# plouj/eraytracer

Measured on AMD Instinct MI355X. Metric: Mpixels/sec at 4096x4096, recursion depth 5 (frame rendered into HBM, gathered to rank 0), higher is better.
Workload: dtype f64; 1 GPU; S64 4096x4096 depth 5; scene=s64, spp=1, width=4096, height=4096, depth=5, order=exact, framebuffer=f32, row_block=16, inflight=4, engine=wave, parallelism=rows1, world_size=1, rccl_ranks=1, hw_queues=4, spheres=64, triangles=0

## Files before the change

### eraytracer_amd/csrc/rt_render.hip

```cpp
#pragma clang fp contract(off)

#include <hip/hip_runtime.h>

#include <chrono>
#include <cmath>
#include <cstddef>
#include <cstdio>
#include <cstdlib>
#include <cstring>
#include <algorithm>
#include <mutex>
#include <type_traits>
#include <vector>

#include "../../include/rt_mi355x.h"
#include "rt_layout.h"
#include "rt_internal.h"
#include "rt_scene.h"

using namespace rtl;

namespace {

constexpr int BLOCK = 256;
// ... 437 lines not shown

}

size_t rt_trim(rt_prepared *p) {
    if (!p) return 0;
    DevGuard g(p->device);
    const size_t freed = free_work(p);
    p->pmask_valid = false;
    ++p->gen;
    return freed;
}

namespace {

size_t queue_budget() {
    static size_t b = [] {
        const char *s = std::getenv("RT_QUEUE_MB");
        size_t mb = s ? std::strtoull(s, nullptr, 10) : 8192;
        return (mb < 64 ? 64 : mb) << 20;
    }();
    return b;
}

bool lit_overlap(const rt_prepared *p) {
    static bool env_on = [] {
        const char *s = std::getenv("RT_LIT_STREAM");
        return !(s && std::strcmp(s, "0") == 0);
    }();
    return p->side_mode < 0 ? env_on : p->side_mode != 0;
}

int side_stream(rt_prepared *p, int depth) {
    if (!p->side[0]) {
        int least = 0, greatest = 0;
        HIPCHK(hipDeviceGetStreamPriorityRange(&least, &greatest));
        for (hipStream_t &x : p->side) HIPCHK(hipStreamCreateWithPriority(&x, hipStreamNonBlocking, least));
    }
    while (p->ev_level.size() < (size_t)depth + 1) {
        hipEvent_t a = nullptr, b = nullptr;
        HIPCHK(hipEventCreateWithFlags(&a, hipEventDisableTiming));
        if (hipEventCreateWithFlags(&b, hipEventDisableTiming) != hipSuccess) {
            (void)hipEventDestroy(a);
            return RT_EHIP;
        }
        p->ev_level.push_back(a);
        p->ev_lit.push_back(b);
    }
    return RT_OK;
}

size_t valid_slab_rows(int H, int rb, int sh, int ns) {
    const size_t slab = rt_shard_rows((uint32_t)H, (uint32_t)rb, (uint32_t)ns);
    size_t v = 0;
    for (size_t blk = 0; blk * rb < slab; ++blk) {
        const long long base = ((long long)blk * ns + sh) * rb;
        v += (size_t)std::max(0LL, std::min((long long)rb, (long long)H - base));
    }
    return v;
}

bool wave_single_write(const rt_prepared *p, int D, bool levels) {
    const int nrefl = (p->hdr.n_light > 0 && D > 1) ? D - 1 : 0;
    const bool overlap = lit_overlap(p) && D > 1 && p->hdr.n_light > 0;
    return nrefl == 0 || (!overlap && !levels);
}

template <int PREC, bool GENPOW>
int launch_wavefront(rt_prepared *p, int W, int H, int D, int rb, int sh, int ns, int row_begin, int row_end, void *out,
                     uint8_t *levels, hipStream_t st, int spp = 1, int sample = 0, unsigned long long seed = 0,
                     double *acc = nullptr, int levels_hit = 0) {
    uint8_t *const levels_primary = levels;
    if (levels_hit) levels = nullptr;
    const int slab_rows = row_end - row_begin;
    const int nlev = D > 0 ? D : 1;
    const size_t per_row = (size_t)W * nlev * sizeof(HitRec);
    int pass_rows = (int)std::min<size_t>((size_t)slab_rows, std::max<size_t>(TILE, queue_budget() / per_row));
    pass_rows = std::max(TILE, pass_rows / TILE * TILE);
    if (pass_rows > slab_rows) pass_rows = slab_rows;
    const int tiles_x = (W + TILE - 1) / TILE;
    const size_t max_tiles = (size_t)tiles_x * ((pass_rows + TILE - 1) / TILE);
    const size_t slots = max_tiles * TILE_SLOTS;
    int rc = grow(p, rt_prepared::W_QUEUE, slots * nlev * sizeof(HitRec));
    const size_t col_doubles = slots * COL_W * (size_t)std::max(1, nlev - 1);
    if (rc == RT_OK) rc = grow(p, rt_prepared::W_COLBUF, col_doubles * sizeof(double));
    if (rc == RT_OK) rc = grow(p, rt_prepared::W_CHILD, slots * nlev);
    if (rc == RT_OK) rc = grow(p, rt_prepared::W_LIT, slots * nlev * sizeof(unsigned));
    if (rc == RT_OK) rc = grow(p, rt_prepared::W_COUNTS, max_tiles * nlev * sizeof(int));
    const bool overlap = lit_overlap(p) && D > 1 && p->hdr.n_light > 0;
    const size_t list0 = level_counts(nlev);
    const size_t items_ints = list0 + slots * nlev;
    if (rc == RT_OK) rc = grow(p, rt_prepared::W_ITEMS, items_ints * sizeof(int));
    if (rc == RT_OK && overlap) rc = side_stream(p, D);
    if (rc != RT_OK) return rc;
    const unsigned long long *pmask = nullptr;
    if (p->hdr.beam_ok && D > 0) {
        const int slab_all = (int)rt_shard_rows(H, rb, ns);
        const size_t nhalf = (size_t)tiles_x * ((slab_all + TILE - 1) / TILE) * 2;
        const long long key[8] = {W, H, rb, sh, ns, spp > 1, (long long)p->scene_gen, slab_all};
        if (!(p->pmask_valid && std::memcmp(key, p->pmask_key, sizeof(key)) == 0)) {
            p->pmask_valid = false;
            ++p->gen;
            if ((rc = grow(p, rt_prepared::W_PMASK, nhalf * p->hdr.n_chunk * 8)) != RT_OK) return rc;
            const dim3 pg((unsigned)std::min<size_t>(4096, (nhalf + 3) / 4));
            KtScope kt(p, RT_KT_PMASK, st);
            with_bool(spp > 1, [&](auto ss) {
                hipLaunchKernelGGL(k_pmask<decltype(ss)::value>, pg, dim3(256), 0, st, p->hdr, p->d_tab, p->d_itab, W, H,
                                   rb, sh, ns, slab_all, (int)nhalf, p->buf<unsigned long long>(rt_prepared::W_PMASK));
            });
            HIPCHK(hipGetLastError());
            std::memcpy(p->pmask_key, key, sizeof(key));
            p->pmask_valid = true;
        }
        pmask = p->buf<unsigned long long>(rt_prepared::W_PMASK);
    }
    auto ls = [&](int k) { return overlap ? p->side[std::min(k, 1)] : st; };
    HitRec *const q = p->buf<HitRec>(rt_prepared::W_QUEUE);
    double *const d_colbuf = p->buf<double>(rt_prepared::W_COLBUF);
    uint8_t *const d_child = p->buf<uint8_t>(rt_prepared::W_CHILD);
    unsigned *const d_lit = p->buf<unsigned>(rt_prepared::W_LIT);
    int *const d_counts = p->buf<int>(rt_prepared::W_COUNTS);
    int *const d_items = p->buf<int>(rt_prepared::W_ITEMS);
    const int nrefl = (p->hdr.n_light > 0 && D > 1) ? D - 1 : 0;
    const int nshade = D > 0 ? 1 + nrefl : 0;
    const bool sph_only = p->hdr.n_tri == 0 && p->hdr.n_pl == 0 && p->hdr.cull_ok && p->hdr.occ_ok;
    const bool staged = sph_only && p->hdr.l_bytes > 0;
    const size_t lds = staged ? (size_t)p->hdr.l_bytes : 0;
    SceneHdr rhdr = p->hdr;
    size_t lds_bvh = lds;
    if (rhdr.bvh_ok) {
        const size_t nb = (size_t)rhdr.n_bvh * BVH_NODE_DOUBLES * 8, sb = (size_t)rhdr.n_sph * SPH_W * 8;
        if (nb + sb <= (size_t)BVH_LDS_MAX) {
            rhdr.l_bvh = (int)lds_bvh;
            rhdr.l_bsph = (int)(lds_bvh + nb);
            lds_bvh += nb + sb;
        }
        rhdr.l_stack = (int)lds_bvh;
        lds_bvh += (size_t)BLOCK * rhdr.bvh_depth * sizeof(unsigned);
    }
    auto bvh_at = [&](int k) { return !staged && rhdr.bvh_ok && k >= rhdr.bvh_level; };
    auto lds_r = [&](int k) { return bvh_at(k) ? lds_bvh : lds; };
    const bool fuse = !overlap && !levels && nrefl > 0;
    const bool iw = fuse && p->hdr.n_light <= 32 && nrefl >= 2;
    for (int row0 = row_begin; row0 < row_end; row0 += pass_rows) {
        const int rows = std::min(pass_rows, row_end - row0);
        const int ntiles = tiles_x * ((rows + TILE - 1) / TILE);
        const size_t off = (size_t)row0 * W;
        void *o = static_cast<char *>(out) + off * 3 * (PREC == RT_OUT_F64 ? 8 : 4);
        uint8_t *lv = levels ? levels + off : nullptr;
        uint8_t *lv0 = levels_primary ? levels_primary + off : nullptr;
        double *acc_p = acc ? acc + off * 3 : nullptr;
        auto qk = [&](int k) { return q + (size_t)k * ntiles * TILE_SLOTS; };
        auto ck = [&](int k) { return d_counts + (size_t)k * ntiles; };
        int *nitems = d_items;
        int *lists = d_items + list0;
        auto ik = [&](int k) { return lists + (size_t)k * ntiles * TILE_SLOTS; };
        auto colk = [&](int k) { return k > 0 ? d_colbuf + (size_t)(k - 1) * ntiles * TILE_SLOTS * COL_W : nullptr; };
        auto chk = [&](int k) { return d_child + (size_t)k * ntiles * TILE_SLOTS; };
        auto litk = [&](int k) { return d_lit + (size_t)k * ntiles * TILE_SLOTS; };
        const dim3 iblocks((ntiles + ITEMS_BLOCK - 1) / ITEMS_BLOCK);
        const PassGeom g{W, H, rb, sh, ns, row0, spp, sample, seed, acc_p};
        const dim3 grid(std::min(ntiles, PRIMARY_GRID));
        {
            KtScope kt(p, RT_KT_PRIMARY, st);
            with_bool(lv0 != nullptr, [&](auto has_lv) {
                hipLaunchKernelGGL((k_primary<PREC, decltype(has_lv)::value>), grid, dim3(PRIMARY_BLOCK), 0, st, p->hdr,
                                   p->d_tab, p->d_itab, W, H, D, rb, sh, ns, rows, row0, o, lv0, q, d_counts, ntiles, spp,
                                   sample, seed, acc_p, pmask, nitems);
            });
        }
        HIPCHK(hipGetLastError());
        const int sblocks = std::min<int>(STRIDE_BLOCKS, (ntiles * (TILE_SLOTS / 64) + BLOCK / 64 - 1) / (BLOCK / 64));
        const int sblocks1 = std::min<int>(STRIDE_BLOCKS_L1, (ntiles * (TILE_SLOTS / 64) + BLOCK / 64 - 1) / (BLOCK / 64));
        const int sblocksw = std::min<int>(STRIDE_BLOCKS_WALK, (ntiles * (TILE_SLOTS / 64) + BLOCK / 64 - 1) / (BLOCK / 64));
        const int sblocksb = std::min<int>(STRIDE_BLOCKS_BVH, (ntiles * (TILE_SLOTS / 64) + BLOCK / 64 - 1) / (BLOCK / 64));
        auto level_lists = [&](int k) -> int {
            if (iw && k == nrefl) return RT_OK;
            hipLaunchKernelGGL(k_items, iblocks, dim3(ITEMS_BLOCK), 0, st, ck(k), ntiles, ik(k), nitems + k);
            HIPCHK(hipGetLastError());
            if (overlap) {
                HIPCHK(hipEventRecord(p->ev_level[k], st));
                HIPCHK(hipStreamWaitEvent(ls(k), p->ev_level[k], 0));
            }
            if (fuse && k < nrefl) return RT_OK;
            if (k == nrefl && k >= 2) {
                if (overlap) HIPCHK(hipEventRecord(p->ev_lit[k], ls(k)));
                return RT_OK;
            }
            const int lblocks = k >= 2 ? std::min(sblocks, DEEP_LIGHT_BLOCKS) : sblocks;
            with_sph(staged, sph_only, [&](auto sph) {
                hipLaunchKernelGGL((k_light<PREC, GENPOW, decltype(sph)::value>), dim3(lblocks), dim3(BLOCK), lds, ls(k),
                                   p->hdr, p->d_tab, p->d_itab, k, o, qk(k), ik(k), nitems + k, colk(k), litk(k), g);
            });
            HIPCHK(hipGetLastError());
            if (overlap) HIPCHK(hipEventRecord(p->ev_lit[k], ls(k)));
            return RT_OK;
        };
        if (nshade > 0 && (rc = level_lists(0)) != RT_OK) return rc;
        for (int k = 1; k <= nrefl; ++k) {
            KtScope kt(p, k == 1 ? RT_KT_LEVEL1 : 0, st);
            if (fuse) {
                const bool bvh_k = bvh_at(k), ilp = bvh_k || k != 1, last = ilp && iw && k == nrefl;
                with_sph(staged, sph_only, [&](auto sph) {
                    constexpr int SPH = decltype(sph)::value;
                    auto rs = [&](auto ilp_c, auto bvh_c, auto last_c) {
                        constexpr bool BVH = decltype(bvh_c)::value;
                        hipLaunchKernelGGL(
                            (k_reflect_shade<PREC, GENPOW, SPH, decltype(ilp_c)::value, BVH, decltype(last_c)::value>),
                            dim3(k == 1 ? sblocks1 : BVH ? sblocksb : sblocks), dim3(BLOCK), lds_r(k), st, rhdr, p->d_tab,
                            p->d_itab, k, o, qk(k - 1), ik(k - 1), nitems + (k - 1), qk(k), ck(k), iw ? nullptr : chk(k - 1),
                            colk(k - 1), g, iw && k >= 2 ? (k == nrefl ? 2 : 1) : 0);
                    };
                    auto rs_ilp = [&](auto bvh_c) {
                        with_bool(last, [&](auto last_c) { rs(std::true_type{}, bvh_c, last_c); });
                    };
                    if (!ilp) rs(std::false_type{}, std::false_type{}, std::false_type{});
                    else if constexpr (SPH == 2) rs_ilp(std::false_type{});
                    else with_bool(bvh_k, rs_ilp);
                });
            } else {
                with_bool(lv != nullptr, [&](auto has_lv) {
                    with_bool(k != 1, [&](auto ilp_c) {
                        hipLaunchKernelGGL((k_reflect<decltype(has_lv)::value, decltype(ilp_c)::value>), dim3(sblocks),
                                           dim3(BLOCK), lds, st, rhdr, p->d_tab, p->d_itab, k, qk(k - 1), ik(k - 1),
                                           nitems + (k - 1), qk(k), ck(k), lv, chk(k - 1), g);
                    });
                });
            }
            HIPCHK(hipGetLastError());
            if ((rc = level_lists(k)) != RT_OK) return rc;
        }
        if (nrefl > 0) {
            const size_t ls_ = (size_t)ntiles * TILE_SLOTS;
            const bool bits = p->hdr.n_light <= 32;
            auto walk = [&](hipStream_t s_, int lo, int hi, bool deep) {
                with_sph(staged, sph_only, [&](auto sph) {
                    with_bool(bits, [&](auto bits_c) {
                        auto launch = [&](auto deep_c, auto pad_c) {
                            hipLaunchKernelGGL((k_walk<PREC, GENPOW, decltype(sph)::value, decltype(bits_c)::value,
                                                       decltype(deep_c)::value, decltype(pad_c)::value>),
                                               dim3(sblocksw), dim3(BLOCK), lds, s_, p->hdr, p->d_tab, p->d_itab, D, o, q,
                                               ls_, lists, nitems, d_colbuf, d_child, d_lit, lo, hi, g);
                        };
                        if (deep && fuse && bits) launch(std::true_type{}, std::true_type{});
                        else if (deep) launch(std::true_type{}, std::false_type{});
                        else launch(std::false_type{}, std::false_type{});
                    });
                });
            };
            if (overlap) {
                HIPCHK(hipStreamWaitEvent(p->side[0], p->ev_lit[1], 0));
                if (D > 2) HIPCHK(hipStreamWaitEvent(p->side[0], p->ev_level[2], 0));
                walk(p->side[0], 1, 2, false);
                HIPCHK(hipGetLastError());
                HIPCHK(hipEventRecord(p->ev_lit[0], p->side[0]));
            }
            if (D > 2 && overlap) {
                with_sph(staged, sph_only, [&](auto sph) {
                    hipLaunchKernelGGL((k_walk_deep<GENPOW, decltype(sph)::value>), dim3(sblocks), dim3(BLOCK), lds, st,
                                       p->hdr, p->d_tab, p->d_itab, D, q, ls_, lists, nitems, d_child, colk(2));
                });
                HIPCHK(hipGetLastError());
            }
            if (overlap) {
                HIPCHK(hipStreamWaitEvent(st, p->ev_lit[nrefl], 0));
                HIPCHK(hipStreamWaitEvent(st, p->ev_lit[0], 0));
                if (D > 2) walk(st, 2, D, false);
            } else if (!iw) {
                walk(st, 1, D, true);
            }
            HIPCHK(hipGetLastError());
        } else if (overlap && nshade > 0) {
            HIPCHK(hipStreamWaitEvent(st, p->ev_lit[0], 0));
        }
    }
    return RT_OK;
}

bool graphs_on() {
    static bool on = [] {
        const char *s = std::getenv("RT_GRAPH");
        return s && std::strcmp(s, "1") == 0;
    }();
    return on;
}

template <typename F>
int launch_frame(rt_prepared *p, const long long (&args)[12], hipStream_t st, F &&enqueue) {
    hipStreamCaptureStatus cs = hipStreamCaptureStatusNone;
    if (!graphs_on() || hipStreamIsCapturing(st, &cs) != hipSuccess || cs != hipStreamCaptureStatusNone)
        return enqueue(st);
    long long key[12];
    std::memcpy(key, args, sizeof(key));
    key[11] = (long long)p->gen;
// ... 184 lines not shown
```

### eraytracer_amd/csrc/rt_shade.inc

```

#ifndef RT_MAX_GROUPS
#define RT_MAX_GROUPS 3
#endif
constexpr int MAX_GROUPS = RT_MAX_GROUPS;
constexpr int UNION_CHUNKS = 4;
template <bool PRE, bool ILP = false, int SPH = 0, bool NB = false>
__device__ __forceinline__ int nearest(const Scene &S, int org, const D3 &o, const D3 &d, double &bt, bool act,
                                       int grp = -1, bool bvh = false) {
    const SceneHdr &h = S.h;
    bt = __builtin_inf();
    int bid = 0x7fffffff;
    if (__ballot(act) == 0) return -1;
    const double A4 = 4 * (d.x * d.x + d.y * d.y + d.z * d.z);
    RT_STAT(PRE ? ST_NEAR_PRE : ST_NEAR_GEN, 1);
    RT_STAT(ST_NEAR_LANES, __popcll(__ballot(act)));
    if constexpr (NB) {
        for (int chunk = 0; chunk < h.n_sph; chunk += 64)
            scan_spheres<PRE, ILP, (SPH >= 1)>(S, org, o, d, A4, chunk, chunk_all(h.n_sph, chunk), bt, bid);
        scan_tri_pl<PRE>(S, org, o, d, bt, bid);
        return (act && bid != 0x7fffffff) ? bid : -1;
    }
    if (!PRE && bvh) {
        if (h.l_bvh >= 0 && h.l_bsph >= 0)
            scan_bvh<true, true, (SPH >= 1)>(S, o, d, A4, act, bt, bid);
// ... 213 lines not shown
                          ts);
        } else {
            const double *p = S.tab + h.o_pl + loc * PL_W;
            valid = pl_t(D3{p[0], p[1], p[2]}, sd, S.tab[h.o_pl_org + org * h.n_pl + loc], ts);
        }
    }
    bool blocked = !valid;
    if (__all(blocked)) return false;
    const bool sph_targets = SPH || (h.occ_ok && __ballot(!blocked && kind != K_SPHERE) == 0);
    double tmax = __builtin_inf();
    Beam b;
    b.on = false;
    if (!SPH && !NB && !sph_targets) b = shadow_cone(hb, Lp, tmax);
    RT_STAT(ST_SHADOW, 1);
    RT_STAT(ST_SHADOW_CONE_ON, (sph_targets || b.on) ? 1 : 0);
    for (int chunk = 0; chunk < h.n_sph; chunk += 64) {
        unsigned long long m;
        if (sph_targets) {
            const unsigned long long *occ = occ_masks<SPH>(S, light, chunk >> 6);
            const int ncell = SPH == 2 ? 1 : h.occ_cells;
            unsigned long long mine = blocked ? 0ull : occ[(loc * ncell + cell) * h.n_chunk];
            for (;;) {
                const bool w = !blocked && mine != 0;
                if (__ballot(w) == 0) break;
                const int lk = w ? __builtin_ctzll(mine) : 0, k = chunk + lk;
                mine &= mine - 1;
                RT_STAT(ST_SHADOW_ITER, 1);
                const double2 *q = reinterpret_cast<const double2 *>(org_row<SPH>(S, org, chunk)) + 2 * lk;
                const double2 q01 = q[0], q23 = q[1];
                const double B = 2 * (sd.x * q01.x + sd.y * q01.y + sd.z * q23.x);
                double t;
                const bool hit = sph_t_wave<(SPH >= 1)>(B, q23.y, A4, t);
                bool blk = w & hit & (t < ts);
                if (__ballot(t == ts) != 0) blk = blk | (w & hit & (t == ts) & (sph_id<SPH>(S, k) < c));
                blocked = blocked | blk;
            }
            if (__all(blocked)) return false;
            continue;
        } else if (!SPH) {
            m = (!NB && b.on) ? cull_chunk(S, b, chunk, org, tmax) : chunk_all(h.n_sph, chunk);
            if (skip >= chunk && skip < chunk + 64) m &= ~(1ull << (skip - chunk));
        }
        RT_STAT(ST_SHADOW_CAND, __popcll(m));
        while (!SPH && m) {
            const int k = chunk + __builtin_ctzll(m);
            m &= m - 1;
            RT_STAT(ST_SHADOW_ITER, 1);
            const double *q = S.tab + h.o_sph_org + (org * h.n_sph + k) * SPH_ORG_W;
            const int id = S.itab[h.i_sph_id + k];
            const double B = 2 * (sd.x * q[0] + sd.y * q[1] + sd.z * q[2]);
            double t;
            const bool hit = sph_t_wave(B, q[3], A4, t);
            blocked = blocked | (hit & ((t < ts) | ((t == ts) & (id < c))));
            if (__all(blocked)) return false;
        }
    }
    if (SPH) return !blocked;
    for (int k = 0; k < h.n_tri; ++k) {
        if (!blocked) {
            const double *g = S.tab + h.o_tri + k * TRI_W;
            const double *q = S.tab + h.o_tri_org + (org * h.n_tri + k) * TRI_ORG_W;
            double t;
            if (tri_t(sd, D3{g[3], g[4], g[5]}, D3{g[6], g[7], g[8]}, D3{q[0], q[1], q[2]}, D3{q[3], q[4], q[5]}, t)) {
                int id = S.itab[h.i_tri_id + k];
                blocked = t < ts || (t == ts && id < c);
            }
        }
        if (__all(blocked)) return false;
    }
    for (int k = 0; k < h.n_pl; ++k) {
        if (!blocked) {
            const double *p = S.tab + h.o_pl + k * PL_W;
            double t;
            if (pl_t(D3{p[0], p[1], p[2]}, sd, S.tab[h.o_pl_org + org * h.n_pl + k], t)) {
                int id = S.itab[h.i_pl_id + k];
                blocked = t < ts || (t == ts && id < c);
            }
        }
        if (__all(blocked)) return false;
    }
    return !blocked;
}

template <bool GENPOW, int SPH = 0, bool NB = false, bool OPQ = false>
__device__ __forceinline__ D3 shade(const Scene &S, int id, const D3 &d, const D3 &hit, const D3 &N, const D3 &col,
                                    double refl, bool active, unsigned *bits = nullptr) {
    const SceneHdr &h = S.h;
    if (__ballot(active) == 0) return D3{0.0, 0.0, 0.0};
    const Target T = make_target<SPH>(S, id, active);
    HitBall hb;
    hb.on = false;
    hb.cx = hb.cy = hb.cz = hb.r = 0.0;
    if (!SPH && !NB && (!h.occ_ok || __ballot(active && T.kind != K_SPHERE) != 0)) hb = make_hitball(h, active, hit);
    RT_STAT(ST_SHADE, 1);
    D3 F = {0.0, 0.0, 0.0};
    for (int i = 0; i < h.n_light; ++i) {
        const Scene &SL = S;
        const double *L = SL.tab + SL.h.o_light + i * LIGHT_W;
        int idl = id;
        asm volatile("" : "+v"(idl));
        const double *m = obj_row<SPH>(S, idl);
        const D3 Lc = {L[0], L[1], L[2]}, Lp = {L[3], L[4], L[5]}, Sc = {L[6], L[7], L[8]};
        const double2 m34 = *reinterpret_cast<const double2 *>(m + 4), m67 = *reinterpret_cast<const double2 *>(m + 6);
        const D3 mc = {m[3], m34.x, m34.y};
        const double spow = m67.x, shin = m67.y;
        const D3 ln = normalize3(D3{Lp.x - hit.x, Lp.y - hit.y, Lp.z - hit.z}, SPH && SL.h.norm_ok);
        const double dd = max0(dot3(N, ln));
        const D3 diff = {mc.x * dd, mc.y * dd, mc.z * dd};
        const D3 hn = normalize3(D3{ln.x + -d.x, ln.y + -d.y, ln.z + -d.z});
        const double sp = shin * pow_libm<GENPOW>(max0(dot3(hn, N)), spow, active);
        const D3 spec = {Sc.x * sp, Sc.y * sp, Sc.z * sp};
        const D3 con = {diff.x + spec.x, diff.y + spec.y, diff.z + spec.z};
        const D3 lc = {Lc.x * con.x, Lc.y * con.y, Lc.z * con.z};
        const bool need = active && !(lc.x == 0.0 && lc.y == 0.0 && lc.z == 0.0);
        const bool lb = lit_by<SPH, NB>(SL, i, T, D3{-ln.x, -ln.y, -ln.z}, need, hb, Lp);
        if (bits && lb && i < 32) *bits |= 1u << i;
        const double lit = lb ? 1.0 : 0.0;
        D3 c = col;
        if (OPQ) asm volatile("" : "+v"(c.x), "+v"(c.y), "+v"(c.z));
        F.x = F.x + (c.x * refl + lc.x * lit);
        F.y = F.y + (c.y * refl + lc.y * lit);
        F.z = F.z + (c.z * refl + lc.z * lit);
    }
    return F;
}
```

### eraytracer_amd/csrc/rt_wave.inc

```

struct HitRec {
    double hx, hy, hz;
    double dx, dy, dz;
    int pix;
    int obj;
    int parent;
    int pbits;
};
static_assert(sizeof(HitRec) == 64, "HitRec is one 64-byte record");
static_assert(offsetof(HitRec, parent) == 56 && offsetof(HitRec, pbits) == 60, "HitRec: (parent, pbits) in one 8-byte word");

struct Rec0 {
    int pix;
    int obj;
    double t;
};
static_assert(sizeof(Rec0) == 16, "Rec0 is one 16-byte record");

struct PassGeom {
    int W, H, rb, shard, nshards, row0, spp, sample;
    unsigned long long seed;
    double *acc;
};

// ... 447 lines not shown
                                                   const int *__restrict__ nhits_prev, HitRec *__restrict__ q_k,
                                                   int *__restrict__ cnt_k, uint8_t *__restrict__ levels,
                                                   uint8_t *__restrict__ child_prev, PassGeom g) {
    const Scene S{hdr, tab, itab};
    for_hits(idx_prev, nhits_prev, [&](int slot, bool act, int) {
        RT_STAT(ST_WAVES, 1);
        const HitRec r = k == 1 ? load_rec0(hdr, g, q_prev, slot) : q_prev[slot];
        const D3 h = {r.hx, r.hy, r.hz};
        const D3 N = hit_normal<0>(S, r.obj, h);
        reflect_record<LEVELS, ILP>(S, k, r, slot, act, h, N, q_k, cnt_k, levels, child_prev);
    });
}

#ifdef RT_DEBUG_LISTS
#define RT_LINK_CHECK(cond, ...)                                                                                   \
    do {                                                                                                           \
        if (!(cond)) {                                                                                             \
            printf(__VA_ARGS__);                                                                                   \
            __builtin_trap();                                                                                      \
        }                                                                                                          \
    } while (0)
#else
#define RT_LINK_CHECK(cond, ...)                                                                                   \
    do {                                                                                                           \
    } while (0)
#endif

template <bool GENPOW, int SPH = 0>
__device__ __forceinline__ D3 shade_bits(const Scene &S, int id, const D3 &d, const D3 &hit, const D3 &N, const D3 &col,
                                         double refl, unsigned bits) {
    const SceneHdr &h = S.h;
    const double *m = obj_row<SPH>(S, id);
    D3 F = {0.0, 0.0, 0.0};
    for (int i = 0; i < h.n_light; ++i) {
        const double *L = S.tab + h.o_light + i * LIGHT_W;
        const D3 Lc = {L[0], L[1], L[2]}, Lp = {L[3], L[4], L[5]}, Sc = {L[6], L[7], L[8]};
        const double2 m34 = *reinterpret_cast<const double2 *>(m + 4), m67 = *reinterpret_cast<const double2 *>(m + 6);
        const D3 mc = {m[3], m34.x, m34.y};
        const double spow = m67.x, shin = m67.y;
        const D3 ln = normalize3(D3{Lp.x - hit.x, Lp.y - hit.y, Lp.z - hit.z}, SPH && h.norm_ok);
        const double dd = max0(dot3(N, ln));
        const D3 diff = {mc.x * dd, mc.y * dd, mc.z * dd};
        const D3 hn = normalize3(D3{ln.x + -d.x, ln.y + -d.y, ln.z + -d.z});
        const double sp = shin * pow_libm<GENPOW>(max0(dot3(hn, N)), spow);
        const D3 spec = {Sc.x * sp, Sc.y * sp, Sc.z * sp};
        const D3 con = {diff.x + spec.x, diff.y + spec.y, diff.z + spec.z};
        const D3 lc = {Lc.x * con.x, Lc.y * con.y, Lc.z * con.z};
        const double lit = ((bits >> i) & 1u) ? 1.0 : 0.0;
        D3 c = col;
        asm volatile("" : "+v"(c.x), "+v"(c.y), "+v"(c.z));
        F.x = F.x + (c.x * refl + lc.x * lit);
        F.y = F.y + (c.y * refl + lc.y * lit);
        F.z = F.z + (c.z * refl + lc.z * lit);
    }
    return F;
}

template <int PREC, bool GENPOW, int SPH>
__device__ __forceinline__ void walk_up(const Scene &S, const PassGeom &g, const HitRec *__restrict__ q,
                                        size_t level_slots, int lv, D3 c, int parent, unsigned pb, int pix, bool on,
                                        void *__restrict__ out) {
    const unsigned long long m = __ballot(on);
    if (m == 0) return;
    const int lead = __builtin_ctzll(m);
    for (int k = lv - 1; k >= 0; --k) {
        RT_LINK_CHECK(!on || (unsigned)parent < (unsigned)level_slots,
                      "walk_up: level %d: parent link %d outside the level's %d slots (pixel %d, from level %d)\n", k,
                      parent, (int)level_slots, pix, lv);
        const int lp = __builtin_amdgcn_readlane(parent, lead);
        int ps = on ? parent : lp;
        ps = (unsigned)ps < (unsigned)level_slots ? ps : 0;
        const HitRec r = k == 0 ? load_rec0(S.h, g, q, ps) : q[(size_t)k * level_slots + ps];
        RT_LINK_CHECK(!on || r.pix == pix, "walk_up: level %d slot %d: parent of pixel %d holds pixel %d\n", k, ps, pix,
                      r.pix);
        const D3 h = {r.hx, r.hy, r.hz};
        c = shade_bits<GENPOW, SPH>(S, r.obj, D3{r.dx, r.dy, r.dz}, h, hit_normal<SPH>(S, r.obj, h), c,
                                    obj_row<SPH>(S, r.obj)[8], pb);
        parent = r.parent;
        pb = (unsigned)r.pbits;
    }
    if (on) put_pixel<PREC>(out, g, (size_t)pix, c);
}

constexpr int COL_W = 4;
__device__ __forceinline__ void put_col_entry(double *col_k, int slot, const D3 &F, const int2 *link) {
    double2 *w = reinterpret_cast<double2 *>(col_k + COL_W * (size_t)slot);
    w[0] = double2{F.x, F.y};
    w[1] = double2{F.z, __builtin_bit_cast(double, *link)};
}
template <int PREC>
__device__ __forceinline__ void put_colour(int k, void *out, double *col_k, const HitRec &r, int slot, const D3 &F,
                                           const PassGeom &g, const int2 *link) {
    if (k > 0) {
        put_col_entry(col_k, slot, F, link);
    } else {
        put_pixel<PREC>(out, g, (size_t)r.pix, F);
    }
}

#ifndef RT_LIGHT_WAVES
#define RT_LIGHT_WAVES 0
#endif
#if RT_LIGHT_WAVES > 0
#define RT_LIGHT_BOUNDS __launch_bounds__(BLOCK, RT_LIGHT_WAVES)
#else
#define RT_LIGHT_BOUNDS __launch_bounds__(BLOCK)
#endif
template <int PREC, bool GENPOW, int SPH>
__global__ RT_LIGHT_BOUNDS void k_light(SceneHdr hdr, const double *__restrict__ tab,
                                                 const int *__restrict__ itab, int k, void *__restrict__ out,
                                                 const HitRec *__restrict__ q_k, const int *__restrict__ idx_k,
                                                 const int *__restrict__ nhits_k, double *__restrict__ col_k,
                                                 unsigned *__restrict__ lit_k, PassGeom g) {
    const Scene S{hdr, tab, itab};
    if (k >= 2 && !deep_dense(nhits_k - k)) return;
    if (no_records_for_block(nhits_k)) return;
    stage_tables<SPH>(S);
    for_hits(idx_k, nhits_k, [&](int slot, bool act, int) {
        const HitRec r = k == 0 ? load_rec0(hdr, g, q_k, slot) : q_k[slot];
        const D3 h = {r.hx, r.hy, r.hz};
        const D3 N = hit_normal<SPH>(S, r.obj, h);
        const double refl = obj_row<SPH>(S, r.obj)[8];
        unsigned bits = 0;
        const D3 F = shade<GENPOW, SPH>(S, r.obj, D3{r.dx, r.dy, r.dz}, h, N, D3{0.0, 0.0, 0.0}, refl, act, &bits);
        if (act) {
            int ls = slot;
            asm volatile("" : "+v"(ls));
            put_colour<PREC>(k, out, col_k, r, slot, F, g, reinterpret_cast<const int2 *>(&q_k[ls].parent));
            lit_k[slot] = bits;
        }
    });
}

#ifndef RT_FUSED_WAVES
#define RT_FUSED_WAVES 5
#endif
#ifndef RT_FUSED_WAVES_SPH
#define RT_FUSED_WAVES_SPH 5
#endif
#ifndef RT_FUSED_WAVES_L2
#define RT_FUSED_WAVES_L2 RT_FUSED_WAVES_SPH
#endif
#ifndef RT_FUSED_WAVES_MIXED
#define RT_FUSED_WAVES_MIXED 4
#endif
#ifndef RT_FUSED_WAVES_MIXED_GENPOW
#define RT_FUSED_WAVES_MIXED_GENPOW 3
#endif
#ifndef RT_FUSED_WAVES_GENPOW
#define RT_FUSED_WAVES_GENPOW 3
#endif
#ifndef RT_LAST_WAVES_SPH
#define RT_LAST_WAVES_SPH 4
#endif
#if RT_FUSED_WAVES > 0
#define RT_FUSED_BOUNDS                                                                                            \
    __launch_bounds__(BLOCK, LAST ? (SPH == 0 && GENPOW ? 2 : SPH == 0 || GENPOW ? 3 : RT_LAST_WAVES_SPH) :    \
                             (SPH == 0 ? (GENPOW ? RT_FUSED_WAVES_MIXED_GENPOW : RT_FUSED_WAVES_MIXED)             \
                                       : GENPOW ? RT_FUSED_WAVES_GENPOW                                            \
                                       : (SPH == 1 && !BVH) ? RT_FUSED_WAVES_L2                                    \
                                                              : (SPH >= 1 && !BVH) ? RT_FUSED_WAVES_SPH            \
                                                                                   : RT_FUSED_WAVES))
#else
#define RT_FUSED_BOUNDS __launch_bounds__(BLOCK)
#endif
template <int PREC, bool GENPOW, int SPH, bool ILP, bool BVH, bool LAST = false>
__global__ RT_FUSED_BOUNDS void k_reflect_shade(SceneHdr hdr, const double *__restrict__ tab,
                                                const int *__restrict__ itab, int k, void *__restrict__ out,
                                                const HitRec *__restrict__ q_prev, const int *__restrict__ idx_prev,
                                                const int *__restrict__ nhits_prev, HitRec *__restrict__ q_k,
                                                int *__restrict__ cnt_k, uint8_t *__restrict__ child_prev,
                                                double *__restrict__ col_prev, PassGeom g, int iw) {
    const Scene S{hdr, tab, itab};
    if (no_records_for_block(nhits_prev)) return;
    stage_tables<SPH>(S);
    if (BVH) stage_bvh(S);
    const bool shade_here = k - 1 < 2 || (ILP && iw != 0) || deep_dense(nhits_prev - (k - 1));
    const bool walk_here = ILP && iw != 0 && shade_here;
    constexpr bool last_here = LAST;
    RT_LINK_CHECK(!LAST || (walk_here && iw == 2), "k_reflect_shade: LAST launched at level %d with iw %d\n", k, iw);
    const size_t lslots = (size_t)(q_k - q_prev);
    const HitRec *q0 = q_prev - (size_t)(k - 1) * lslots;
    auto group = [&](int slot, const HitRec &r, bool act) {
        const Scene SL = fresh_scene(S);
        const D3 h = {r.hx, r.hy, r.hz};
        const D3 N = hit_normal<SPH>(SL, r.obj, h);
        int cs = -1;
        ChildHit ch;
        cs = reflect_record<false, ILP, SPH, BVH>(SL, k, r, slot, act, h, N, q_k, cnt_k, nullptr, child_prev,
                                                  !last_here, LAST ? &ch : nullptr);
        const bool child = cs >= 0;
        const int wslot = child ? cs : slot;
        if (shade_here) {
            const double refl = obj_row<SPH>(SL, r.obj)[8];
            if constexpr (ILP && LAST) {
                if (last_here) {
                    const bool cl = act && child;
                    const unsigned long long cm = __ballot(cl);
                    D3 cc = {0.0, 0.0, 0.0};
                    if (cm) {
                        const int cl_lead = __builtin_ctzll(cm);
                        const D3 hm = {h.x + ch.d.x * ch.t, h.y + ch.d.y * ch.t, h.z + ch.d.z * ch.t};
                        const D3 hl = {readlane_d(hm.x, cl_lead), readlane_d(hm.y, cl_lead), readlane_d(hm.z, cl_lead)};
                        const D3 dl = {readlane_d(ch.d.x, cl_lead), readlane_d(ch.d.y, cl_lead), readlane_d(ch.d.z, cl_lead)};
                        const int il = __builtin_amdgcn_readlane(ch.id, cl_lead);
                        const D3 hc = cl ? hm : hl, dc = cl ? ch.d : dl;
                        const int idc = cl ? ch.id : il;
                        const D3 c1 = shade<GENPOW, SPH>(SL, idc, dc, hc, hit_normal<SPH>(SL, idc, hc), D3{0.0, 0.0, 0.0},
                                                         obj_row<SPH>(SL, idc)[8], cl);
                        if (cl) cc = c1;
                    }
                    const D3 c = shade<GENPOW, SPH, false, true>(SL, r.obj, D3{r.dx, r.dy, r.dz}, h, N, cc, refl, act);
                    walk_up<PREC, GENPOW, SPH>(SL, g, q0, lslots, k - 1, c, r.parent, (unsigned)r.pbits, r.pix, act, out);
                    return;
                }
            }
            unsigned bits = 0;
            const D3 F = shade<GENPOW, SPH>(SL, r.obj, D3{r.dx, r.dy, r.dz}, h, N, D3{0.0, 0.0, 0.0}, refl, act, &bits);
            if constexpr (ILP) {
                if (walk_here) {
                    walk_up<PREC, GENPOW, SPH>(SL, g, q0, lslots, k - 1, F, r.parent, (unsigned)r.pbits, r.pix,
                                               act && !child, out);
                    if (act && child) reinterpret_cast<unsigned *>(q_k + wslot)[15] = bits;
                    return;
                }
            }
            if (act) {
                if (!child) {
                    int ls = slot;
                    asm volatile("" : "+v"(ls));
                    put_colour<PREC>(k - 1, out, col_prev, r, wslot, F, g,
                                     reinterpret_cast<const int2 *>(&q_prev[ls].parent));
                }
                else reinterpret_cast<unsigned *>(q_k + wslot)[15] = bits;
            }
        }
    };
    if (!ILP && SPH == 2) {
        for_rec0_pf(idx_prev, nhits_prev, reinterpret_cast<const Rec0 *>(q_prev), [&](int slot, const Rec0 &r0, bool act, int) {
            group(slot, rec0_to_rec(fresh_scene(S).h, g, r0), act);
        });
    } else {
        for_hits_pf(idx_prev, nhits_prev, [&](int slot, bool act, int, auto &&prefetch) {
            HitRec r;
            if (opq(k) == 1) {
                const Rec0 r0 = reinterpret_cast<const Rec0 *>(q_prev)[slot];
                prefetch();
                r = rec0_to_rec(fresh_scene(S).h, g, r0);
            } else {
                r = q_prev[slot];
                prefetch();
            }
            group(slot, r, act);
        });
    }
}

#ifndef RT_SHADE_WAVES
#define RT_SHADE_WAVES 0
#endif
#ifndef RT_SHADE_WAVES_SPH
#define RT_SHADE_WAVES_SPH 5
#endif
#define RT_SHADE_BOUNDS                                                                                            \
    __launch_bounds__(BLOCK, SPH >= 1 && RT_SHADE_WAVES_SPH > 0 ? (GENPOW ? 4 : RT_SHADE_WAVES_SPH)               \
                                                                 : (RT_SHADE_WAVES > 0 ? RT_SHADE_WAVES : 1))
__device__ __forceinline__ bool level_group(const int *__restrict__ nhits, int lo, int hi, int u, int &j, int &g) {
    g = u;
    for (int i = lo; i < hi; ++i) {
        j = hi - 1 - (i - lo);
        const int ng = (nhits[j] + 63) >> 6;
        if (g < ng) return true;
        g -= ng;
    }
    return false;
}


template <bool GENPOW, int SPH>
__global__ RT_SHADE_BOUNDS void k_walk_deep(SceneHdr hdr, const double *__restrict__ tab,
                                            const int *__restrict__ itab, int depth, const HitRec *__restrict__ q,
                                            size_t level_slots, const int *__restrict__ idx,
                                            const int *__restrict__ nhits, const uint8_t *__restrict__ child,
                                            double *__restrict__ col2) {
    if (deep_dense(nhits)) return;
    const Scene S{hdr, tab, itab};
    const int lane = threadIdx.x & 63;
    int total = 0;
    for (int k = 2; k < depth; ++k) total += (nhits[k] + 63) >> 6;
    if ((long)blockIdx.x * (BLOCK / 64) >= (long)total) return;
    stage_tables<SPH>(S);
    const int nw = gridDim.x * (BLOCK / 64);
    for (int u = blockIdx.x * (BLOCK / 64) + (threadIdx.x >> 6); u < total; u += nw) {
        int j, g;
        level_group(nhits, 2, depth, u, j, g);
        const int p = g * 64 + lane;
        const bool in = p < nhits[j];
        int slot = idx[(size_t)j * level_slots + (in ? p : g * 64)];
        const bool term = in && (j == depth - 1 || !child[(size_t)j * level_slots + slot]);
        if (__ballot(term) == 0) continue;
        HitRec r = q[(size_t)j * level_slots + slot];
        D3 h = {r.hx, r.hy, r.hz};
        D3 c = shade<GENPOW, SPH>(S, r.obj, D3{r.dx, r.dy, r.dz}, h, hit_normal<SPH>(S, r.obj, h), D3{0.0, 0.0, 0.0},
                                  obj_row<SPH>(S, r.obj)[8], term);
        const int lead = __builtin_ctzll(__ballot(term));
// ... 101 lines not shown
```

Baseline: 46170 Mpixels/s.

## Cache per-light diffuse/specular terms during shading and fold them in the walk-up

When shading a hit that spawns a reflected child, the per-light diffuse and specular scalars are stored to a terms buffer that reuses the colour buffer's memory. The final walk back up the ray tree then rebuilds each ancestor's colour from these stored terms instead of recomputing normals, half vectors and pow for every light. This swaps recomputation (notably pow) for extra global stores and loads of double2 per light per slot, and it only applies to staged sphere-only scenes with up to 8 lights.

```diff
diff --git a/eraytracer_amd/csrc/rt_render.hip b/eraytracer_amd/csrc/rt_render.hip
--- a/eraytracer_amd/csrc/rt_render.hip
+++ b/eraytracer_amd/csrc/rt_render.hip
@@ -543,11 +543,19 @@
     const size_t slots = max_tiles * TILE_SLOTS;
     int rc = grow(p, rt_prepared::W_QUEUE, slots * nlev * sizeof(HitRec));
     const size_t col_doubles = slots * COL_W * (size_t)std::max(1, nlev - 1);
-    if (rc == RT_OK) rc = grow(p, rt_prepared::W_COLBUF, col_doubles * sizeof(double));
+    const bool overlap = lit_overlap(p) && D > 1 && p->hdr.n_light > 0;
+    const int nrefl = (p->hdr.n_light > 0 && D > 1) ? D - 1 : 0;
+    const bool fuse = !overlap && !levels && nrefl > 0;
+    const bool iw = fuse && p->hdr.n_light <= 32 && nrefl >= 2;
+    const bool sph_only = p->hdr.n_tri == 0 && p->hdr.n_pl == 0 && p->hdr.cull_ok && p->hdr.occ_ok;
+    const bool staged = sph_only && p->hdr.l_bytes > 0;
+    const bool fold = iw && staged && p->hdr.n_light <= TERM_MAX_LIGHTS;
+    const size_t term_bytes =
+        fold ? slots * (size_t)(nrefl - 1) * term_stride(p->hdr.n_light) * sizeof(double2) : 0;
+    if (rc == RT_OK) rc = grow(p, rt_prepared::W_COLBUF, std::max(col_doubles * sizeof(double), term_bytes));
     if (rc == RT_OK) rc = grow(p, rt_prepared::W_CHILD, slots * nlev);
     if (rc == RT_OK) rc = grow(p, rt_prepared::W_LIT, slots * nlev * sizeof(unsigned));
     if (rc == RT_OK) rc = grow(p, rt_prepared::W_COUNTS, max_tiles * nlev * sizeof(int));
-    const bool overlap = lit_overlap(p) && D > 1 && p->hdr.n_light > 0;
     const size_t list0 = level_counts(nlev);
     const size_t items_ints = list0 + slots * nlev;
     if (rc == RT_OK) rc = grow(p, rt_prepared::W_ITEMS, items_ints * sizeof(int));
@@ -581,10 +589,7 @@
     unsigned *const d_lit = p->buf<unsigned>(rt_prepared::W_LIT);
     int *const d_counts = p->buf<int>(rt_prepared::W_COUNTS);
     int *const d_items = p->buf<int>(rt_prepared::W_ITEMS);
-    const int nrefl = (p->hdr.n_light > 0 && D > 1) ? D - 1 : 0;
     const int nshade = D > 0 ? 1 + nrefl : 0;
-    const bool sph_only = p->hdr.n_tri == 0 && p->hdr.n_pl == 0 && p->hdr.cull_ok && p->hdr.occ_ok;
-    const bool staged = sph_only && p->hdr.l_bytes > 0;
     const size_t lds = staged ? (size_t)p->hdr.l_bytes : 0;
     SceneHdr rhdr = p->hdr;
     size_t lds_bvh = lds;
@@ -600,8 +605,7 @@
     }
     auto bvh_at = [&](int k) { return !staged && rhdr.bvh_ok && k >= rhdr.bvh_level; };
     auto lds_r = [&](int k) { return bvh_at(k) ? lds_bvh : lds; };
-    const bool fuse = !overlap && !levels && nrefl > 0;
-    const bool iw = fuse && p->hdr.n_light <= 32 && nrefl >= 2;
+    double2 *const d_terms = fold ? reinterpret_cast<double2 *>(d_colbuf) : nullptr;
     for (int row0 = row_begin; row0 < row_end; row0 += pass_rows) {
         const int rows = std::min(pass_rows, row_end - row0);
         const int ntiles = tiles_x * ((rows + TILE - 1) / TILE);
@@ -669,7 +673,7 @@
                             (k_reflect_shade<PREC, GENPOW, SPH, decltype(ilp_c)::value, BVH, decltype(last_c)::value>),
                             dim3(k == 1 ? sblocks1 : BVH ? sblocksb : sblocks), dim3(BLOCK), lds_r(k), st, rhdr, p->d_tab,
                             p->d_itab, k, o, qk(k - 1), ik(k - 1), nitems + (k - 1), qk(k), ck(k), iw ? nullptr : chk(k - 1),
-                            colk(k - 1), g, iw && k >= 2 ? (k == nrefl ? 2 : 1) : 0);
+                            colk(k - 1), g, iw && k >= 2 ? (k == nrefl ? 2 : 1) : 0, d_terms);
                     };
                     auto rs_ilp = [&](auto bvh_c) {
                         with_bool(last, [&](auto last_c) { rs(std::true_type{}, bvh_c, last_c); });
diff --git a/eraytracer_amd/csrc/rt_shade.inc b/eraytracer_amd/csrc/rt_shade.inc
--- a/eraytracer_amd/csrc/rt_shade.inc
+++ b/eraytracer_amd/csrc/rt_shade.inc
@@ -319,9 +319,12 @@
     return !blocked;
 }
 
+constexpr int TERM_MAX_LIGHTS = 8;
+__host__ __device__ constexpr int term_stride(int n_light) { return n_light <= 4 ? 4 : 8; }
 template <bool GENPOW, int SPH = 0, bool NB = false, bool OPQ = false>
 __device__ __forceinline__ D3 shade(const Scene &S, int id, const D3 &d, const D3 &hit, const D3 &N, const D3 &col,
-                                    double refl, bool active, unsigned *bits = nullptr) {
+                                    double refl, bool active, unsigned *bits = nullptr, double2 *terms = nullptr,
+                                    int tslot = 0, bool tstore = false) {
     const SceneHdr &h = S.h;
     if (__ballot(active) == 0) return D3{0.0, 0.0, 0.0};
     const Target T = make_target<SPH>(S, id, active);
@@ -346,6 +349,7 @@
         const D3 diff = {mc.x * dd, mc.y * dd, mc.z * dd};
         const D3 hn = normalize3(D3{ln.x + -d.x, ln.y + -d.y, ln.z + -d.z});
         const double sp = shin * pow_libm<GENPOW>(max0(dot3(hn, N)), spow, active);
+        if (terms && active && tstore) terms[(size_t)tslot * term_stride(h.n_light) + i] = double2{dd, sp};
         const D3 spec = {Sc.x * sp, Sc.y * sp, Sc.z * sp};
         const D3 con = {diff.x + spec.x, diff.y + spec.y, diff.z + spec.z};
         const D3 lc = {Lc.x * con.x, Lc.y * con.y, Lc.z * con.z};
diff --git a/eraytracer_amd/csrc/rt_wave.inc b/eraytracer_amd/csrc/rt_wave.inc
--- a/eraytracer_amd/csrc/rt_wave.inc
+++ b/eraytracer_amd/csrc/rt_wave.inc
@@ -553,6 +553,71 @@
     if (on) put_pixel<PREC>(out, g, (size_t)pix, c);
 }
 
+template <int PREC, int SPH>
+__device__ __forceinline__ void walk_fold(const Scene &S, const PassGeom &g, const HitRec *__restrict__ q,
+                                          size_t level_slots, int lv, D3 c, int slot, int parent, unsigned pb, int pix,
+                                          bool on, void *__restrict__ out, const double2 *__restrict__ terms) {
+    const unsigned long long m = __ballot(on);
+    if (m == 0) return;
+    const int lead = __builtin_ctzll(m);
+    const SceneHdr &h = S.h;
+    const int stride = term_stride(h.n_light);
+    for (int k = lv - 1; k >= 0; --k) {
+        RT_LINK_CHECK(!on || (unsigned)parent < (unsigned)level_slots,
+                      "walk_fold: level %d: parent link %d outside the level's %d slots (pixel %d, from level %d)\n", k,
+                      parent, (int)level_slots, pix, lv);
+        RT_LINK_CHECK(!on || (unsigned)slot < (unsigned)level_slots,
+                      "walk_fold: level %d: slot %d outside the level's %d slots (pixel %d, from level %d)\n", k + 1,
+                      slot, (int)level_slots, pix, lv);
+        const int lp = __builtin_amdgcn_readlane(parent, lead), lcs = __builtin_amdgcn_readlane(slot, lead);
+        int ps = on ? parent : lp, cs = on ? slot : lcs;
+        ps = (unsigned)ps < (unsigned)level_slots ? ps : 0;
+        cs = (unsigned)cs < (unsigned)level_slots ? cs : 0;
+        const double2 *e = terms + ((size_t)k * level_slots + cs) * stride;
+        int4 t;
+        if (k == 0) {
+            const Rec0 r0 = reinterpret_cast<const Rec0 *>(q)[ps];
+            t = int4{r0.pix, r0.obj, -1, 0};
+        } else {
+            t = *reinterpret_cast<const int4 *>(&q[(size_t)k * level_slots + ps].pix);
+        }
+        RT_LINK_CHECK(!on || t.x == pix, "walk_fold: level %d slot %d: parent of pixel %d holds pixel %d\n", k, ps, pix,
+                      t.x);
+        const double *mr = obj_row<SPH>(S, t.y);
+        const double refl = mr[8];
+        D3 F = {0.0, 0.0, 0.0};
+        for (int i0 = 0; i0 < h.n_light; i0 += 4) {
+            const double2 e0 = e[i0], e1 = e[i0 + 1], e2 = e[i0 + 2], e3 = e[i0 + 3];
+#pragma unroll
+            for (int j = 0; j < 4; ++j) {
+                const int i = i0 + j;
+                if (i >= h.n_light) break;
+                const double *L = S.tab + h.o_light + i * LIGHT_W;
+                const D3 Lc = {L[0], L[1], L[2]}, Sc = {L[6], L[7], L[8]};
+                const double2 m34 = *reinterpret_cast<const double2 *>(mr + 4);
+                const D3 mc = {mr[3], m34.x, m34.y};
+                const double2 ds = j == 0 ? e0 : j == 1 ? e1 : j == 2 ? e2 : e3;
+                const double dd = ds.x, sp = ds.y;
+                const D3 diff = {mc.x * dd, mc.y * dd, mc.z * dd};
+                const D3 spec = {Sc.x * sp, Sc.y * sp, Sc.z * sp};
+                const D3 con = {diff.x + spec.x, diff.y + spec.y, diff.z + spec.z};
+                const D3 lc = {Lc.x * con.x, Lc.y * con.y, Lc.z * con.z};
+                const double lit = ((pb >> i) & 1u) ? 1.0 : 0.0;
+                D3 cc = c;
+                asm volatile("" : "+v"(cc.x), "+v"(cc.y), "+v"(cc.z));
+                F.x = F.x + (cc.x * refl + lc.x * lit);
+                F.y = F.y + (cc.y * refl + lc.y * lit);
+                F.z = F.z + (cc.z * refl + lc.z * lit);
+            }
+        }
+        c = F;
+        slot = ps;
+        parent = t.z;
+        pb = (unsigned)t.w;
+    }
+    if (on) put_pixel<PREC>(out, g, (size_t)pix, c);
+}
+
 constexpr int COL_W = 4;
 __device__ __forceinline__ void put_col_entry(double *col_k, int slot, const D3 &F, const int2 *link) {
     double2 *w = reinterpret_cast<double2 *>(col_k + COL_W * (size_t)slot);
@@ -641,11 +706,13 @@
                                                 const HitRec *__restrict__ q_prev, const int *__restrict__ idx_prev,
                                                 const int *__restrict__ nhits_prev, HitRec *__restrict__ q_k,
                                                 int *__restrict__ cnt_k, uint8_t *__restrict__ child_prev,
-                                                double *__restrict__ col_prev, PassGeom g, int iw) {
+                                                double *__restrict__ col_prev, PassGeom g, int iw,
+                                                double2 *__restrict__ terms_staged) {
     const Scene S{hdr, tab, itab};
     if (no_records_for_block(nhits_prev)) return;
     stage_tables<SPH>(S);
     if (BVH) stage_bvh(S);
+    double2 *const terms = SPH == 2 ? terms_staged : nullptr;
     const bool shade_here = k - 1 < 2 || (ILP && iw != 0) || deep_dense(nhits_prev - (k - 1));
     const bool walk_here = ILP && iw != 0 && shade_here;
     constexpr bool last_here = LAST;
@@ -682,16 +749,26 @@
                         if (cl) cc = c1;
                     }
                     const D3 c = shade<GENPOW, SPH, false, true>(SL, r.obj, D3{r.dx, r.dy, r.dz}, h, N, cc, refl, act);
-                    walk_up<PREC, GENPOW, SPH>(SL, g, q0, lslots, k - 1, c, r.parent, (unsigned)r.pbits, r.pix, act, out);
+                    if (terms)
+                        walk_fold<PREC, SPH>(SL, g, q0, lslots, k - 1, c, slot, r.parent, (unsigned)r.pbits, r.pix, act, out,
+                                             terms);
+                    else
+                        walk_up<PREC, GENPOW, SPH>(SL, g, q0, lslots, k - 1, c, r.parent, (unsigned)r.pbits, r.pix, act, out);
                     return;
                 }
             }
             unsigned bits = 0;
-            const D3 F = shade<GENPOW, SPH>(SL, r.obj, D3{r.dx, r.dy, r.dz}, h, N, D3{0.0, 0.0, 0.0}, refl, act, &bits);
+            const D3 F = shade<GENPOW, SPH>(SL, r.obj, D3{r.dx, r.dy, r.dz}, h, N, D3{0.0, 0.0, 0.0}, refl, act, &bits,
+                                            terms ? terms + (size_t)(k - 1) * lslots * term_stride(SL.h.n_light) : nullptr,
+                                            wslot, child);
             if constexpr (ILP) {
                 if (walk_here) {
-                    walk_up<PREC, GENPOW, SPH>(SL, g, q0, lslots, k - 1, F, r.parent, (unsigned)r.pbits, r.pix,
-                                               act && !child, out);
+                    if (terms)
+                        walk_fold<PREC, SPH>(SL, g, q0, lslots, k - 1, F, wslot, r.parent, (unsigned)r.pbits, r.pix,
+                                             act && !child, out, terms);
+                    else
+                        walk_up<PREC, GENPOW, SPH>(SL, g, q0, lslots, k - 1, F, r.parent, (unsigned)r.pbits, r.pix,
+                                                   act && !child, out);
                     if (act && child) reinterpret_cast<unsigned *>(q_k + wslot)[15] = bits;
                     return;
                 }
```

Result: faster. 47470 Mpixels/s, median of 6 (+2.8%).
